# PinataFarms/DAD-3DHeads

Hardware: NVIDIA B200
Metric: heads/sec @256x256 (5023-vert FLAME) (higher is better)
Workload: dtype fp32 operands as fp16 hi/lo split (22-bit), 3 tensor-core products, fp32 accumulate (1e-4 contract met; strict 24-bit mode timed under strict_fp32_operands)

## Files before the change

dad_3dheads_b200/csrc/encoder.cu:

```cuda
#include <algorithm>
#include <cmath>
#include <cstdlib>
#include <cstring>
#include <map>
#include <memory>
#include <string>
#include <vector>

#include "../../include/dad3d.h"
#include "common.h"
#include "encoder_kernels.cuh"
#include "tmap.h"

using namespace dad3d;

namespace {

constexpr int kImg = 256;
constexpr int kStageUnits[4] = {3, 4, 6, 3};
constexpr int kNumFilters = 256;
constexpr int kHeat = 68;
constexpr int kHeatCat = 128;
constexpr int kMlpOut = 549;
constexpr float kLimitValue = 3.0f;
// ... 17 lines not shown
  if (cout <= 80) return 80;
  return 96;
}

inline uint16_t host_bf16(float x) {
  uint32_t u;
  std::memcpy(&u, &x, 4);
  if ((u & 0x7f800000u) == 0x7f800000u) return static_cast<uint16_t>(u >> 16);
  u += 0x7fffu + ((u >> 16) & 1u);
  return static_cast<uint16_t>(u >> 16);
}
inline uint16_t host_f16(float x) { return __half_as_ushort(__float2half_rn(x)); }
inline float host_f16_to_f32(uint16_t b) { return __half2float(__ushort_as_half(b)); }
inline float host_bf16_to_f32(uint16_t b) {
  uint32_t u = static_cast<uint32_t>(b) << 16;
  float f;
  std::memcpy(&f, &u, 4);
  return f;
}

struct TensorInfo {
  int N = 0, H = 0, W = 0, C = 0;
  bool f32 = false;
  int planes = 1;
  size_t bytes = 0;
  int first = 1 << 30, last = -1;
  size_t off = 0;
  uint8_t* ptr = nullptr;
  std::string name;
  long long plane_elems() const { return static_cast<long long>(N) * H * W * C; }
};

enum StepKind { kStemConv, kStemS2d, kStemPool, kConv, kFuse, kConcat, kGap, kFinalize, kHeatExport };

struct Step {
  StepKind kind;
  int in = -1, out = -1, res = -1, out_f32 = -1, in2 = -1, in3 = -1;
  const ConvW* w = nullptr;
  int stride = 1, pad = 0, relu = 0, res_mode = 0, res_stride = 1;
  int up2 = 0;
  int parity = 0;
  int variant = 0;
  int sparse_rows = 0;
  int stem = 0;
  GemmMaps maps;
  GemmGeom geom;
  EpiConv::Params epi;
  float fw[3] = {0, 0, 0};
  int nsrc = 0;
};

struct Plan {
  int B = 0;
  void* ws = nullptr;
  size_t ws_bytes = 0;
  std::vector<TensorInfo> tensors;
  std::vector<Step> steps;
  int t_mlp_out = -1, t_heat = -1, t_c4 = -1;
};

}

struct dad3d_encoder {
  int device = 0;
  int num_sms = 0;
  int P = 3;
  int fp16 = 0;
  int n_mma = 6;
  int n_acc = 2;
  int mma_a[kMaxMma], mma_b[kMaxMma], mma_acc[kMaxMma];
  std::map<std::string, ConvW> convs;
  float* d_stem_w = nullptr;
  float* d_stem_b = nullptr;
  float bifpn_w[2][20];
  std::unique_ptr<Plan> plan;
  size_t ws_cache_B = 0, ws_cache_bytes = 0;
  bool stem_simt = false;
  bool use_halo = true;
  int halo_cluster = 1;
  bool kernels_configured = false, stem_configured = false;
  bool td_parity = false;
  bool heat_sparse = true;
  bool use_pair = false;
  bool use_pdl = false;
  bool debug_keep_all = false;
  bool profile = false;
  std::vector<std::pair<cudaEvent_t, cudaEvent_t>> prof_events;
  size_t prof_used = 0;
  std::vector<const void*> prof_steps;
  double prof_flops = 0.0;
  double prof_bytes = 0.0;
};

namespace {

struct Builder {
  dad3d_encoder* enc;
  Plan* plan;
  int B;

  int tensor(int N, int H, int W, int C, bool f32 = false) {
    TensorInfo t;
    t.N = N; t.H = H; t.W = W; t.C = C; t.f32 = f32;
    t.planes = f32 ? 1 : enc->P;
    t.bytes = align_up(static_cast<size_t>(t.plane_elems()) * (f32 ? 4 : 2) * t.planes, 1024);
    plan->tensors.push_back(t);
    return static_cast<int>(plan->tensors.size()) - 1;
  }
  void touch(int t, int step) {
    if (t < 0) return;
    TensorInfo& ti = plan->tensors[t];
    ti.first = std::min(ti.first, step);
    ti.last = std::max(ti.last, step);
  }
  int push(Step s) {
    const int idx = static_cast<int>(plan->steps.size());
    for (int t : {s.in, s.out, s.res, s.out_f32, s.in2, s.in3}) touch(t, idx);
    plan->steps.push_back(s);
    return idx;
  }
  const ConvW* W(const std::string& name) {
    auto it = enc->convs.find(name);
    return it == enc->convs.end() ? nullptr : &it->second;
  }
  int conv(const std::string& name, int in, int stride, int pad, bool relu, int res = -1, int res_mode = 0,
           bool f32_out = false, bool pieces_out = true, int* f32_id = nullptr, int res_stride = 1, bool up2 = false,
           int variant = 0, int reuse_f32 = -1, bool sparse_rows = false) {
    const ConvW* w = W(name);
    const TensorInfo ti = plan->tensors[in];
    const int Ho = (ti.H + 2 * pad - w->R) / stride + 1;
    const int Wo = (ti.W + 2 * pad - w->S) / stride + 1;
    Step s;
    std::memset(&s.maps, 0, sizeof(s.maps));
    s.kind = kConv;
    s.in = in;
    s.w = w;
    s.stride = stride;
    s.pad = pad;
    s.relu = relu ? 1 : 0;
    s.res = res;
    s.res_mode = res_mode;
    s.res_stride = res_stride;
    s.up2 = up2 ? 1 : 0;
    s.out = pieces_out ? tensor(ti.N, up2 ? 2 * Ho : Ho, up2 ? 2 * Wo : Wo, w->cout_pad) : -1;
    s.out_f32 = f32_out ? (reuse_f32 >= 0 ? reuse_f32 : tensor(ti.N, Ho, Wo, w->cout_pad, true)) : -1;
    s.variant = variant;
    s.sparse_rows = sparse_rows ? 1 : 0;
    if (s.out >= 0) plan->tensors[s.out].name = name;
    if (s.out_f32 >= 0) plan->tensors[s.out_f32].name = name + (pieces_out ? ".f32" : "");
    if (f32_id) *f32_id = s.out_f32;
    push(s);
    return s.out;
  }
};

void pick_tile(int Wo, int Ho, int* tw, int* th, int* tn) {
  int w = 1;
  while (w < Wo && w < kBlockM) w <<= 1;
  *tw = w;
  int h = 1;
  while (h < Ho && w * h < kBlockM) h <<= 1;
  *th = h;
  *tn = kBlockM / (w * h);
}

int build_graph(Builder& b) {
  const int B = b.B;
// ... 202 lines not shown
    const TensorInfo& t = plan->tensors[id];
    v.base = reinterpret_cast<const uint16_t*>(t.ptr);
    v.plane = t.plane_elems();
    v.planes = t.planes;
    v.C = t.C;
    return v;
  };
  for (Step& s : plan->steps) {
    if (s.kind != kConv) continue;
    const TensorInfo& ti = plan->tensors[s.in];
    const ConvW* w = s.w;
    const bool src2 = s.res >= 0 && s.res_mode == 4;
    const int cin2 = src2 ? plan->tensors[s.res].C : 0;
    if (!s.stem && ti.C + cin2 != w->cin_pad) {
      set_error("layer " + w->name + ": input has " + std::to_string(ti.C) + "+" + std::to_string(cin2) +
                " channels, weights expect " + std::to_string(w->cin_pad));
      return DAD3D_ERR_INVALID;
    }
    const int Ho = s.stem ? ti.H : s.parity ? ti.H / 2 : (ti.H + 2 * s.pad - w->R) / s.stride + 1;
    const int Wo = s.stem ? ti.W - kS2dPadW : s.parity ? ti.W / 2 : (ti.W + 2 * s.pad - w->S) / s.stride + 1;
    GemmGeom& g = s.geom;
    std::memset(&g, 0, sizeof(g));
    pick_tile(Wo, Ho, &g.tw, &g.th, &g.tn);
    bool halo = enc->use_halo && !s.stem && w->R == 3 && w->S == 3 && s.stride == 1 && s.pad == 1 && Wo >= kHaloTW &&
                Ho >= kHaloTH;
    if (halo) {
      GemmGeom probe;
      std::memset(&probe, 0, sizeof(probe));
      probe.nA = enc->P; probe.nB = enc->P; probe.block_n = w->block_n;
      halo = gemm_halo_b_stages(probe) >= 2;
    }
    if (s.sparse_rows) halo = false;
    if (halo) { g.tw = kHaloTW; g.th = kHaloTH; g.tn = 1; }
    g.tiles_w = ceil_div(Wo, g.tw);
    g.tiles_h = ceil_div(Ho, g.th);
    if (s.sparse_rows) {
      g.tw = Wo; g.th = 2; g.tn = 1;
      if (g.tw * g.th != kBlockM) { set_error("sparse heat rows need a 64-pixel-wide map"); return DAD3D_ERR_INVALID; }
      g.tiles_w = 1;
      const int Hd = plan->tensors[plan->t_c4].H;
      g.rowmap_n = 0;
      for (int i = 0; i < Hd && g.rowmap_n < 32; ++i) {
        const float fy = (Hd > 1) ? i * (static_cast<float>(Ho - 1) / static_cast<float>(Hd - 1)) : 0.f;
        const int y0 = static_cast<int>(fy);
        if (g.rowmap_n == 0 || g.rowmap[g.rowmap_n - 1] != y0) g.rowmap[g.rowmap_n++] = static_cast<unsigned char>(y0);
      }
      g.tiles_h = g.rowmap_n;
    }
    g.tiles_n = ceil_div(ti.N, g.tn);
    g.Wo = Wo; g.Ho = Ho; g.Nimg = ti.N;
    g.stride = s.stride;
    g.R = w->R; g.S = w->S; g.pad_h = s.pad; g.pad_w = s.pad;
    g.cin_blocks = ti.C / kBlockK;
    if (s.stem) { g.cin_blocks = 1; g.pad_h = 2; g.pad_w = 0; }
    if (s.parity) { g.pad_h = -((s.parity - 1) >> 1); g.pad_w = -((s.parity - 1) & 1); }
    g.cl_m = 1; g.cl_n = 1;
    const bool res_in_k = s.res >= 0 && s.res_mode == 1 && w->has_identity;
    const int m_tiles = g.tiles_w * g.tiles_h * g.tiles_n;
    const bool narrow = w->has_b64 && m_tiles * (w->cout_pad / w->block_n) * 2 <= enc->num_sms;
    const int block_n = narrow ? 64 : w->block_n;
    g.block_n = block_n;
    g.n_tiles = w->cout_pad / block_n;
    g.nA = enc->P; g.nB = enc->P;
    g.n_mma = enc->n_mma;
    g.n_acc = enc->n_acc;
    for (int i = 0; i < enc->n_mma; ++i) { g.mma_a[i] = enc->mma_a[i]; g.mma_b[i] = enc->mma_b[i]; g.mma_acc[i] = enc->mma_acc[i]; }
    g.fmt16 = enc->fp16 ? 0u : 1u;
    if (res_in_k) {
      g.res_kb = block_n / kBlockK;
      g.n_mma_res = enc->P;
      for (int i = 0; i < enc->P; ++i) {
        g.mma_res_a[i] = enc->P - 1 - i;
        g.mma_res_acc[i] = (enc->n_acc == 2 && g.mma_res_a[i] != 0) ? 1 : 0;
      }
    }
    if (src2) {
      g.res_kb = cin2 / kBlockK;
      g.res_kind = 1;
      g.res_stride = s.res_stride;
    }
    const bool pair = enc->use_pair && block_n == 128 && w->has_b64 &&
                      ((m_tiles + 1) / 2) * g.n_tiles >= enc->num_sms / 2;
    g.pair = (pair && !halo) ? 1 : 0;
    g.stages = gemm_max_stages(g);
    if (halo) {
      g.halo = 1;
      if (enc->halo_cluster == 2 && block_n == 128 && w->has_b64 && m_tiles >= 2 * enc->num_sms) {
        g.cl_m = 2;
        g.sched = 1;
      }
      g.stages = 2;
      g.stages_b = gemm_halo_b_stages(g);
      if (g.stages_b < 2) { set_error("layer " + w->name + ": halo pipeline does not fit shared memory"); return DAD3D_ERR_INVALID; }
    }
    if (g.stages < 2) { set_error("layer " + w->name + ": pipeline does not fit shared memory"); return DAD3D_ERR_INVALID; }
    for (int p = 0; p < enc->P; ++p) {
      const uint64_t dims[4] = {static_cast<uint64_t>(s.stem ? kBlockK : ti.C), static_cast<uint64_t>(s.stem ? Wo : ti.W),
                                static_cast<uint64_t>(ti.H), static_cast<uint64_t>(ti.N)};
      const uint64_t strides[3] = {static_cast<uint64_t>(ti.C) * 2, static_cast<uint64_t>(ti.W) * ti.C * 2,
                                   static_cast<uint64_t>(ti.H) * ti.W * ti.C * 2};
      const uint32_t box[4] = {kBlockK, static_cast<uint32_t>(halo ? kHaloPW : g.tw * s.stride),
                               static_cast<uint32_t>(halo ? kHaloPH : g.th * s.stride), static_cast<uint32_t>(g.tn)};
      const uint32_t es[4] = {1, static_cast<uint32_t>(s.stride), static_cast<uint32_t>(s.stride), 1};
      const uint16_t* basep = reinterpret_cast<const uint16_t*>(ti.ptr) + static_cast<size_t>(p) * ti.plane_elems();
      if (!make_tmap_16bit(&s.maps.a[p], basep, 4, dims, strides, box, es)) return DAD3D_ERR_CUDA;
      s.maps.b[p] = (narrow || g.pair || g.cl_m == 2) ? w->map_b64[p] : w->map_b[p];
    }
    if (res_in_k || src2) {
      const TensorInfo& tr = plan->tensors[s.res];
      const int rs = src2 ? s.res_stride : 1;
      for (int p = 0; p < enc->P; ++p) {
        const uint64_t dims[4] = {static_cast<uint64_t>(tr.C), static_cast<uint64_t>(tr.W), static_cast<uint64_t>(tr.H),
                                  static_cast<uint64_t>(tr.N)};
        const uint64_t strides[3] = {static_cast<uint64_t>(tr.C) * 2, static_cast<uint64_t>(tr.W) * tr.C * 2,
                                     static_cast<uint64_t>(tr.H) * tr.W * tr.C * 2};
        const uint32_t box[4] = {kBlockK, static_cast<uint32_t>(g.tw * rs), static_cast<uint32_t>(g.th * rs),
                                 static_cast<uint32_t>(g.tn)};
        const uint32_t es[4] = {1, static_cast<uint32_t>(rs), static_cast<uint32_t>(rs), 1};
        const uint16_t* basep = reinterpret_cast<const uint16_t*>(tr.ptr) + static_cast<size_t>(p) * tr.plane_elems();
        if (!make_tmap_16bit(&s.maps.r[p], basep, 4, dims, strides, box, es)) return DAD3D_ERR_CUDA;
      }
    }
    EpiConv::Params& ep = s.epi;
    std::memset(&ep, 0, sizeof(ep));
    ep.bias = w->d_bias;
    ep.scale = w->d_scale;
    ep.relu = s.relu;
    ep.res_mode = (res_in_k || src2) ? 0 : s.res_mode;
    ep.res = view(s.res);
    ep.up2 = s.up2;
    ep.parity = s.parity;
    if (s.res >= 0 && !src2 && plan->tensors[s.res].C != w->cout_pad) {
      set_error("layer " + w->name + ": residual channel mismatch");
      return DAD3D_ERR_INVALID;
    }
    if (s.out >= 0) {
      const TensorInfo& to = plan->tensors[s.out];
      ep.out = reinterpret_cast<uint16_t*>(to.ptr);
      ep.out_plane = to.plane_elems();
      ep.out_planes = to.planes;
      ep.ld_out = to.C;
      if (block_n != 64 && block_n != 128) {
        set_error("layer " + w->name + ": piece outputs need block_n 64 or 128");
        return DAD3D_ERR_INVALID;
      }
      const int nc = 32;
      const int bw = std::min(g.tw, 32);
      const int bh = std::min(g.th, 32 / bw);
      const int bn = 32 / (bw * bh);
      for (int p = 0; p < to.planes; ++p) {
        uint16_t* basep = reinterpret_cast<uint16_t*>(to.ptr) + static_cast<size_t>(p) * to.plane_elems();
        if (s.up2 || s.parity) {
          const uint64_t C2 = static_cast<uint64_t>(to.C) * 2;
          const uint64_t dims[5] = {static_cast<uint64_t>(to.C), 2, static_cast<uint64_t>(Wo), 2,
                                    static_cast<uint64_t>(to.N) * Ho};
          const uint64_t strides[4] = {C2, 2 * C2, static_cast<uint64_t>(to.W) * C2, 2 * static_cast<uint64_t>(to.W) * C2};
          const uint32_t box[5] = {static_cast<uint32_t>(nc), 1, static_cast<uint32_t>(bw), 1, static_cast<uint32_t>(bh * bn)};
          if (!make_tmap_16bit(&s.maps.c[p], basep, 5, dims, strides, box, nullptr, nc * 2)) return DAD3D_ERR_CUDA;
          continue;
        }
        const uint64_t dims[4] = {static_cast<uint64_t>(to.C), static_cast<uint64_t>(to.W), static_cast<uint64_t>(to.H),
                                  static_cast<uint64_t>(to.N)};
        const uint64_t strides[3] = {static_cast<uint64_t>(to.C) * 2, static_cast<uint64_t>(to.W) * to.C * 2,
                                     static_cast<uint64_t>(to.H) * to.W * to.C * 2};
        const uint32_t box[4] = {static_cast<uint32_t>(nc), static_cast<uint32_t>(bw), static_cast<uint32_t>(bh),
                                 static_cast<uint32_t>(bn)};
// ... 46 lines not shown
      cudaEvent_t a, b;
      DAD3D_CUDA_OK(cudaEventCreate(&a));
      DAD3D_CUDA_OK(cudaEventCreate(&b));
      enc->prof_events.emplace_back(a, b);
    }
    if (enc->prof_steps.size() <= enc->prof_used) enc->prof_steps.resize(enc->prof_used + 1);
    enc->prof_steps[enc->prof_used] = &s;
    ev = &enc->prof_events[enc->prof_used++];
    enc->prof_flops += conv_useful_flops(s);
    DAD3D_CUDA_OK(cudaEventRecord(ev->first, stream));
  }
  {
    cudaLaunchConfig_t cfg{};
    cfg.gridDim = dim3(grid);
    cfg.blockDim = dim3(kGemmThreads);
    cfg.dynamicSmemBytes = gemm_smem_bytes(g);
    cfg.stream = stream;
    cudaLaunchAttribute attr[2];
    int na = 0;
    if (enc->use_pdl) {
      attr[na].id = cudaLaunchAttributeProgrammaticStreamSerialization;
      attr[na].val.programmaticStreamSerializationAllowed = 1;
      ++na;
    }
    if (csz > 1) {
      attr[na].id = cudaLaunchAttributeClusterDimension;
      attr[na].val.clusterDim.x = static_cast<unsigned>(csz);
      attr[na].val.clusterDim.y = 1;
      attr[na].val.clusterDim.z = 1;
      ++na;
    }
    cfg.attrs = attr;
    cfg.numAttrs = na;
    if (g.pair) {
      if (enc->fp16) DAD3D_CUDA_OK(cudaLaunchKernelEx(&cfg, tile_gemm_kernel<EpiConvH, true>, s.maps, g, s.epi));
      else DAD3D_CUDA_OK(cudaLaunchKernelEx(&cfg, tile_gemm_kernel<EpiConv, true>, s.maps, g, s.epi));
    } else {
      if (enc->fp16) DAD3D_CUDA_OK(cudaLaunchKernelEx(&cfg, tile_gemm_kernel<EpiConvH>, s.maps, g, s.epi));
      else DAD3D_CUDA_OK(cudaLaunchKernelEx(&cfg, tile_gemm_kernel<EpiConv>, s.maps, g, s.epi));
    }
  }
  count_launch();
  if (ev) DAD3D_CUDA_OK(cudaEventRecord(ev->second, stream));
  DAD3D_CUDA_OK(cudaGetLastError());
  return DAD3D_OK;
}

}

extern "C" {

int dad3d_encoder_create(dad3d_encoder** out, const dad3d_conv_weights* layers, int32_t n_layers,
                         const float* bifpn_fusion_w_h, int32_t pieces, int32_t operand_format, int32_t device) {
  DAD3D_REQUIRE(out && layers && bifpn_fusion_w_h, "null pointer");
  DAD3D_REQUIRE(pieces >= 1 && pieces <= 3, "pieces must be 1 (one product), 2 (hi/lo, 3 products) or 3 (bf16x3, 6 products)");
  DAD3D_REQUIRE(operand_format == DAD3D_OPERAND_BF16 || (operand_format == DAD3D_OPERAND_FP16 && pieces <= 2),
                "operand_format must be DAD3D_OPERAND_BF16, or DAD3D_OPERAND_FP16 with 1 or 2 pieces");
  DAD3D_CUDA_OK(cudaSetDevice(device));
  cudaDeviceProp prop;
  DAD3D_CUDA_OK(cudaGetDeviceProperties(&prop, device));
  if (prop.major != 10) {
    set_error("libdad3d requires an sm_100 (Blackwell) device");
    return DAD3D_ERR_UNSUPPORTED;
  }
  std::unique_ptr<dad3d_encoder> enc(new dad3d_encoder());
  enc->device = device;
  enc->num_sms = prop.multiProcessorCount;
  enc->P = pieces;
  enc->fp16 = operand_format == DAD3D_OPERAND_FP16 ? 1 : 0;
  if (pieces == 1) {
    enc->n_mma = 1; enc->n_acc = 1; enc->mma_a[0] = 0; enc->mma_b[0] = 0; enc->mma_acc[0] = 0;
  } else if (pieces == 2) {
    const int pa[3] = {1, 0, 0}, pb[3] = {0, 1, 0}, pc[3] = {1, 1, 0};
    enc->n_mma = 3; enc->n_acc = 2;
    for (int i = 0; i < 3; ++i) { enc->mma_a[i] = pa[i]; enc->mma_b[i] = pb[i]; enc->mma_acc[i] = pc[i]; }
  } else {
    const int pa[6] = {2, 0, 1, 1, 0, 0}, pb[6] = {0, 2, 1, 0, 1, 0}, pc[6] = {1, 1, 1, 1, 1, 0};
    enc->n_mma = 6; enc->n_acc = 2;
    for (int i = 0; i < 6; ++i) { enc->mma_a[i] = pa[i]; enc->mma_b[i] = pb[i]; enc->mma_acc[i] = pc[i]; }
  }
  std::memcpy(enc->bifpn_w, bifpn_fusion_w_h, sizeof(enc->bifpn_w));
  {
    const char* e = std::getenv("DAD3D_PDL");
    enc->use_pdl = (e && e[0] == '1');
    const char* e4 = std::getenv("DAD3D_HALO");
    enc->use_halo = !(e4 && e4[0] == '0');
    const char* e5 = std::getenv("DAD3D_HALO_CLUSTER");
    enc->halo_cluster = (e5 && e5[0] == '2') ? 2 : 1;
    const char* e6 = std::getenv("DAD3D_TD_PARITY");
    enc->td_parity = (e6 && e6[0] == '1');
    const char* e9 = std::getenv("DAD3D_HEAT_SPARSE");
    enc->heat_sparse = !(e9 && std::atoi(e9) == 0);
    const char* e3 = std::getenv("DAD3D_PAIR");
    enc->use_pair = (e3 && e3[0] == '1');
    const char* e2 = std::getenv("DAD3D_STEM_SIMT");
    enc->stem_simt = (e2 && e2[0] == '1');
  }

  auto fail = [&](int code) { dad3d_encoder_destroy(enc.release()); return code; };
  std::vector<float> stem_w4;
  for (int li = 0; li < n_layers; ++li) {
    dad3d_conv_weights L = layers[li];
    if (!L.name || !L.weight_h || !L.bias_h || L.cout <= 0 || L.cin <= 0 || L.R <= 0 || L.S <= 0) {
      set_error("invalid layer record " + std::to_string(li));
      return fail(DAD3D_ERR_INVALID);
    }
    const std::string name(L.name);
    if (name == "stem") {
      if (L.cout != 64 || L.cin != 3 || L.R != 7 || L.S != 7) { set_error("stem must be 7x7 3->64"); return fail(DAD3D_ERR_INVALID); }
      std::vector<float> w(147 * 64);
      for (int o = 0; o < 64; ++o)
        for (int r = 0; r < 7; ++r)
          for (int s = 0; s < 7; ++s)
            for (int c = 0; c < 3; ++c)
              w[((c * 7 + r) * 7 + s) * 64 + o] = L.weight_h[((static_cast<size_t>(o) * 7 + r) * 7 + s) * 3 + c];
      if (cudaMalloc(&enc->d_stem_w, w.size() * 4) != cudaSuccess || cudaMalloc(&enc->d_stem_b, 64 * 4) != cudaSuccess ||
          cudaMemcpy(enc->d_stem_w, w.data(), w.size() * 4, cudaMemcpyHostToDevice) != cudaSuccess ||
          cudaMemcpy(enc->d_stem_b, L.bias_h, 64 * 4, cudaMemcpyHostToDevice) != cudaSuccess) {
        set_error("stem upload failed");
        return fail(DAD3D_ERR_CUDA);
      }
      stem_w4.assign(static_cast<size_t>(64) * 4 * 64, 0.f);
      for (int o = 0; o < 64; ++o)
        for (int r = 0; r < 4; ++r)
          for (int dx = 0; dx < 4; ++dx)
            for (int py = 0; py < 2; ++py)
              for (int px = 0; px < 2; ++px) {
                const int ky = 2 * r + py - 1, kx = 2 * dx + px - 1;
                if (ky < 0 || ky > 6 || kx < 0 || kx > 6) continue;
                for (int c = 0; c < 3; ++c)
                  stem_w4[(static_cast<size_t>(o) * 4 + r) * 64 + dx * 16 + (py * 2 + px) * 3 + c] =
                      L.weight_h[((static_cast<size_t>(o) * 7 + ky) * 7 + kx) * 3 + c];
              }
      L.weight_h = stem_w4.data();
      L.cin = 64; L.R = 4; L.S = 1;
    }
    ConvW cw;
    cw.name = name;
    cw.cout = L.cout; cw.cin = L.cin; cw.R = L.R; cw.S = L.S;
    cw.block_n = pick_block_n(L.cout);
    cw.cout_pad = ceil_div(L.cout, cw.block_n) * cw.block_n;
    cw.cin_pad = ceil_div(L.cin, kBlockK) * kBlockK;
    cw.has_identity = name.size() > 4 && L.R == 1 && L.S == 1 &&
                      ((name.compare(name.size() - 2, 2, "c3") == 0 && name.compare(name.size() - 4, 4, "u1c3") != 0) ||
                       name.compare(name.size() - 2, 2, "td") == 0);
    const size_t ktot_main = static_cast<size_t>(L.R) * L.S * cw.cin_pad;
    const size_t ktot = ktot_main + (cw.has_identity ? cw.cout_pad : 0);
    const size_t plane = static_cast<size_t>(cw.cout_pad) * ktot;
    std::vector<uint16_t> packed(plane * pieces, 0);
    std::vector<float> scale(cw.cout_pad, 1.f), up(cw.cout_pad, 1.f);
    if (enc->fp16)
      for (int o = 0; o < L.cout; ++o) {
        float amax = 0.f;
        const float* row = L.weight_h + static_cast<size_t>(o) * L.R * L.S * L.cin;
        for (size_t i = 0; i < static_cast<size_t>(L.R) * L.S * L.cin; ++i) amax = std::max(amax, std::fabs(row[i]));
        int e = 0;
        if (amax > 0.f && std::isfinite(amax)) {
          std::frexp(amax, &e);
          e = std::min(15, 15 - e);
          e = std::max(e, -100);
        }
        up[o] = std::ldexp(1.f, e);
        scale[o] = std::ldexp(1.f, -e);
      }
    if (cw.has_identity)
      for (int o = 0; o < cw.cout_pad; ++o)
        packed[static_cast<size_t>(o) * ktot + ktot_main + o] = enc->fp16 ? host_f16(up[o]) : static_cast<uint16_t>(0x3F80);
    for (int o = 0; o < L.cout; ++o)
      for (int t = 0; t < L.R * L.S; ++t)
        for (int c = 0; c < L.cin; ++c) {
          float r = L.weight_h[(static_cast<size_t>(o) * L.R * L.S + t) * L.cin + c] * up[o];
          const size_t idx = static_cast<size_t>(o) * ktot + static_cast<size_t>(t) * cw.cin_pad + c;
          for (int p = 0; p < pieces; ++p) {
            const uint16_t h = enc->fp16 ? host_f16(r) : host_bf16(r);
            packed[p * plane + idx] = h;
            r -= enc->fp16 ? host_f16_to_f32(h) : host_bf16_to_f32(h);
          }
// ... 288 lines not shown
```

dad_3dheads_b200/csrc/tile_gemm.cuh:

```cuda
#pragma once
#include "ptx.cuh"

namespace dad3d {

constexpr int kBlockM = 128;
constexpr int kBlockK = 64;
constexpr int kTileABytes = kBlockM * kBlockK * 2;
constexpr int kMaxPieces = 3;
constexpr int kMaxMma = 6;
constexpr int kEpiWarps = 8;
constexpr int kFirstEpiWarp = 2;
constexpr int kGemmThreads = (kFirstEpiWarp + kEpiWarps) * 32;
constexpr int kTmemCols = 512;
constexpr int kStageOutBytes = 4096;
constexpr int kGemmSmemLimit = 227 * 1024;
constexpr int kHaloTW = 8, kHaloTH = 16, kHaloPW = kHaloTW + 2, kHaloPH = kHaloTH + 2;
constexpr int kHaloBytes = kHaloPW * kHaloPH * kBlockK * 2;
constexpr int kHaloPieceBytes = 23 * 1024;

struct GemmGeom {
  int tw, th, tn;
  int tiles_w, tiles_h, tiles_n;
  int Wo, Ho, Nimg;
  int stride;
  int R, S, pad_h, pad_w;
  int cin_blocks;
  int n_tiles;
  int block_n;
  int nA, nB;
  int n_mma;
  int mma_a[kMaxMma], mma_b[kMaxMma];
  int n_acc;
  int mma_acc[kMaxMma];
  int res_kb;
  int res_kind;
  int res_stride;
  int n_mma_res;
  int mma_res_a[kMaxPieces], mma_res_acc[kMaxPieces];
  int stages;
  unsigned fmt16;
  int cl_m, cl_n;
  int halo;
  int stages_b;
  int pair;
  int rowmap_n;
  unsigned char rowmap[32];
  int sched;
};

struct GemmMaps {
  CUtensorMap a[kMaxPieces];
  CUtensorMap b[kMaxPieces];
  CUtensorMap c[kMaxPieces];
  CUtensorMap r[kMaxPieces];
};

__host__ __device__ inline int gemm_stage_bytes(const GemmGeom& g) {
  return g.nA * kTileABytes + g.nB * (g.block_n >> g.pair) * kBlockK * 2;
}
__host__ __device__ inline int gemm_halo_a_stage_bytes(const GemmGeom& g) { return g.nA * kHaloPieceBytes; }
__host__ __device__ inline int gemm_b_stage_bytes(const GemmGeom& g) { return g.nB * g.block_n * kBlockK * 2; }
__host__ inline int gemm_fixed_smem_bytes(int extra = 0) {
  return kEpiWarps * kStageOutBytes + extra + 1024  + 512 ;
}
__host__ inline int gemm_max_stages(const GemmGeom& g, int extra = 0) {
  int s = (kGemmSmemLimit - gemm_fixed_smem_bytes(extra)) / gemm_stage_bytes(g);
  return s > 8 ? 8 : s;
}
__host__ inline int gemm_halo_b_stages(const GemmGeom& g, int a_stages = 2) {
  int s = (kGemmSmemLimit - gemm_fixed_smem_bytes(0) - a_stages * gemm_halo_a_stage_bytes(g)) / gemm_b_stage_bytes(g);
  return s > 8 ? 8 : s;
}
__host__ inline int gemm_smem_bytes(const GemmGeom& g, int extra = 0) {
  if (g.halo) return g.stages * gemm_halo_a_stage_bytes(g) + g.stages_b * gemm_b_stage_bytes(g) + gemm_fixed_smem_bytes(extra);
  return g.stages * gemm_stage_bytes(g) + gemm_fixed_smem_bytes(extra);
}

struct TileCoord {
  int m_tile, n_tile;
  int n0, h0, w0;
};

__device__ __forceinline__ TileCoord decode_tile(const GemmGeom& g, int m_tile, int n_tile) {
  TileCoord c;
  c.n_tile = n_tile;
  c.m_tile = m_tile;
  int iw = c.m_tile % g.tiles_w;
  int ih = (c.m_tile / g.tiles_w) % g.tiles_h;
  int in = c.m_tile / (g.tiles_w * g.tiles_h);
  c.n0 = in * g.tn;
  c.h0 = g.rowmap_n > 0 ? static_cast<int>(g.rowmap[ih]) : ih * g.th;
  c.w0 = iw * g.tw;
  return c;
}

__device__ __forceinline__ bool tile_at(const GemmGeom& g, int i, TileCoord* tc) {
  const int m_tiles = g.tiles_w * g.tiles_h * g.tiles_n;
  int m, n;
  if (g.pair) {
    const int t = static_cast<int>(blockIdx.x >> 1) + i * static_cast<int>(gridDim.x >> 1);
    if (t >= ((m_tiles + 1) >> 1) * g.n_tiles) return false;
    n = t % g.n_tiles;
    m = (t / g.n_tiles) * 2 + static_cast<int>(ptx::cluster_ctarank());
  } else if (g.sched == 0) {
    const int t = static_cast<int>(blockIdx.x) + i * static_cast<int>(gridDim.x);
    if (t >= m_tiles * g.n_tiles) return false;
    n = t % g.n_tiles;
    m = t / g.n_tiles;
  } else if (g.cl_m * g.cl_n == 1) {
    m = static_cast<int>(blockIdx.x) + (i / g.n_tiles) * static_cast<int>(gridDim.x);
    if (m >= m_tiles) return false;
    n = i % g.n_tiles;
  } else {
    const int csize = g.cl_m * g.cl_n;
    const int rank = static_cast<int>(ptx::cluster_ctarank());
    const int n_super = (g.n_tiles + g.cl_n - 1) / g.cl_n;
    const int m_super = (m_tiles + g.cl_m - 1) / g.cl_m;
    const int ms = static_cast<int>(blockIdx.x) / csize + (i / n_super) * (static_cast<int>(gridDim.x) / csize);
    if (ms >= m_super) return false;
    m = ms * g.cl_m + rank / g.cl_n;
    n = (i % n_super) * g.cl_n + rank % g.cl_n;
  }
  *tc = decode_tile(g, m, n);
  return true;
}

struct EpiCtx {
  const GemmGeom* g;
  const GemmMaps* maps;
  TileCoord tc;
  int wq;
  int grp;
  int lane;
  uint32_t t_acc;
  uint8_t* stage;
  uint8_t* extra;
  int prev_m_tile;
  mutable int store_seq;
  uint64_t* tempty;
  uint32_t tempty_cluster;
  int n, h, w;
  bool valid;
  long long pix;
  int col0;
  int bw0, bh0, bn0;
};

template <int OFF, int N>
__device__ __forceinline__ void epi_load32(const EpiCtx& c, int c0, float (&x)[N]) {
  static_assert(OFF + 32 <= N, "slice out of range");
  float v[32];
  ptx::tmem_ld_32x32b_x32_f(c.t_acc + static_cast<uint32_t>(c0), v);
  if (c.g->n_acc == 2) {
    float v2[32];
    ptx::tmem_ld_32x32b_x32_f(c.t_acc + static_cast<uint32_t>(c.g->block_n + c0), v2);
    ptx::tmem_ld_wait();
#pragma unroll
    for (int j = 0; j < 32; ++j) x[OFF + j] = v[j] + v2[j];
  } else {
    ptx::tmem_ld_wait();
#pragma unroll
    for (int j = 0; j < 32; ++j) x[OFF + j] = v[j];
  }
}
template <int OFF, int N>
__device__ __forceinline__ void epi_load16(const EpiCtx& c, int c0, float (&x)[N]) {
  static_assert(OFF + 16 <= N, "slice out of range");
  float v[16];
  ptx::tmem_ld_32x32b_x16_f(c.t_acc + static_cast<uint32_t>(c0), v);
  if (c.g->n_acc == 2) {
    float v2[16];
    ptx::tmem_ld_32x32b_x16_f(c.t_acc + static_cast<uint32_t>(c.g->block_n + c0), v2);
    ptx::tmem_ld_wait();
#pragma unroll
    for (int j = 0; j < 16; ++j) x[OFF + j] = v[j] + v2[j];
  } else {
    ptx::tmem_ld_wait();
#pragma unroll
    for (int j = 0; j < 16; ++j) x[OFF + j] = v[j];
  }
}
__device__ __forceinline__ void epi_release_tmem(const EpiCtx& c) {
  ptx::tc_fence_before();
  if (c.tempty_cluster) ptx::mbar_arrive_cluster(c.tempty_cluster);
  else ptx::mbar_arrive(c.tempty);
}
__device__ __forceinline__ void epi_chunk_range(const GemmGeom& g, int grp, int* cb, int* ce) {
  const int nch = (g.block_n + 31) / 32;
  const int per = (nch + 1) / 2;
  *cb = grp * per;
  *ce = min(nch, *cb + per);
}

template <class Epi, bool kPair = false>
__global__ void __launch_bounds__(kGemmThreads, 1)
tile_gemm_kernel(const __grid_constant__ GemmMaps maps, const GemmGeom g, const typename Epi::Params ep) {
  extern __shared__ uint8_t smem_raw[];
  uint8_t* smem = smem_raw + ((1024u - (ptx::smem_u32(smem_raw) & 1023u)) & 1023u);
  const int stage_bytes = g.halo ? gemm_halo_a_stage_bytes(g) : gemm_stage_bytes(g);
  const int b_stage_bytes = gemm_b_stage_bytes(g);
  uint8_t* smem_b = smem + g.stages * stage_bytes;
  uint8_t* out_stage = smem_b + (g.halo ? g.stages_b * b_stage_bytes : 0);
  uint8_t* extra_smem = out_stage + kEpiWarps * kStageOutBytes;
  uint64_t* bars = reinterpret_cast<uint64_t*>(extra_smem + Epi::kExtraSmemBytes);
  uint64_t* full_bar = bars;
  uint64_t* empty_bar = bars + g.stages;
  uint64_t* tfull_bar = bars + 2 * g.stages;
  uint64_t* tempty_bar = tfull_bar + 2;
  uint32_t* tmem_slot = reinterpret_cast<uint32_t*>(tempty_bar + 2);
  uint64_t* bfull_bar = tempty_bar + 3;
  uint64_t* bempty_bar = bfull_bar + 8;

  const int warp = __shfl_sync(0xffffffffu, static_cast<int>(threadIdx.x >> 5), 0);
  const int lane = threadIdx.x & 31;
  const int num_kb = g.R * g.S * g.cin_blocks;

  if (warp == 0 && lane == 0) {
    for (int i = 0; i < g.nA; ++i) ptx::prefetch_tmap(&maps.a[i]);
    for (int i = 0; i < g.nB; ++i) ptx::prefetch_tmap(&maps.b[i]);
  }
  if (warp == 1 && lane == 0) {
    const int n_peers = g.cl_m + g.cl_n - 1;
    for (int s = 0; s < g.stages; ++s) {
      ptx::mbar_init(&full_bar[s], 1);
      ptx::mbar_init(&empty_bar[s], (kPair || g.halo) ? 1 : n_peers);
    }
    if (g.halo)
      for (int s = 0; s < g.stages_b; ++s) {
        ptx::mbar_init(&bfull_bar[s], 1);
        ptx::mbar_init(&bempty_bar[s], g.cl_m);
      }
    for (int b = 0; b < 2; ++b) {
      ptx::mbar_init(&tfull_bar[b], 1);
      ptx::mbar_init(&tempty_bar[b], (kPair ? 2 : 1) * kEpiWarps * 32);
    }
    ptx::fence_mbar_init();
  }
  if (warp == 0) {
    if constexpr (kPair) {
      ptx::tmem_alloc_2sm(tmem_slot, kTmemCols);
      ptx::tmem_relinquish_2sm();
    } else {
      ptx::tmem_alloc(tmem_slot, kTmemCols);
      ptx::tmem_relinquish();
    }
  }
  ptx::tc_fence_before();
  __syncthreads();
  ptx::tc_fence_after();
  const uint32_t tmem_base = *tmem_slot;
  const int csize = kPair ? 2 : g.cl_m * g.cl_n;
  const int crank = csize > 1 ? static_cast<int>(ptx::cluster_ctarank()) : 0;
  const int ci = crank / g.cl_n, cj = crank % g.cl_n;
  uint16_t mask_a = 0, mask_b = 0;
  for (int j = 0; j < g.cl_n; ++j) mask_a |= static_cast<uint16_t>(1u << (ci * g.cl_n + j));
  for (int i = 0; i < g.cl_m; ++i) mask_b |= static_cast<uint16_t>(1u << (i * g.cl_n + cj));
  const uint16_t mask_peers = mask_a | mask_b;
  if (csize > 1) ptx::cluster_sync_all();
  ptx::grid_dep_launch();
  ptx::grid_dep_wait();

  if (warp == 0) {
    if (g.halo) {
      int sa = 0, sbi = 0;
      uint32_t pha = 0, phb = 0;
      auto issue_a = [&](const TileCoord& t, int cb) {
        ptx::mbar_wait(&empty_bar[sa], pha ^ 1u);
        if (ptx::elect_one_sync()) {
          ptx::mbar_expect_tx(&full_bar[sa], static_cast<uint32_t>(g.nA * kHaloBytes));
          for (int i = 0; i < g.nA; ++i)
            ptx::tma_load_4d(smem + sa * stage_bytes + i * kHaloPieceBytes, &maps.a[i], &full_bar[sa], cb * kBlockK, t.w0 - 1,
                             t.h0 - 1, t.n0);
        }
        __syncwarp();
// ... 49 lines not shown
              uint8_t* sb2 = st + g.nA * kTileABytes;
              if (g.res_kind == 0) {
                if (crank == 0)
                  ptx::mbar_expect_tx(&full_bar[stage], static_cast<uint32_t>(2 * (g.nA * kTileABytes + b_half)));
                const int rc = tc.n_tile * g.block_n + r * kBlockK;
                for (int i = 0; i < g.nA; ++i)
                  ptx::tma_load_4d_2sm(st + i * kTileABytes, &maps.r[i], lead_full, rc, tc.w0, tc.h0, tc.n0);
                ptx::tma_load_2d_2sm(sb2, &maps.b[0], lead_full, num_kb * kBlockK + rc, b_row);
              } else {
                if (crank == 0) ptx::mbar_expect_tx(&full_bar[stage], 2 * tx_bytes);
                for (int i = 0; i < g.nA; ++i)
                  ptx::tma_load_4d_2sm(st + i * kTileABytes, &maps.r[i], lead_full, r * kBlockK, tc.w0 * g.res_stride,
                                       tc.h0 * g.res_stride, tc.n0);
                for (int i = 0; i < g.nB; ++i)
                  ptx::tma_load_2d_2sm(sb2 + i * b_half, &maps.b[i], lead_full, (num_kb + r) * kBlockK, b_row);
              }
            } else if (g.res_kind == 0) {
              ptx::mbar_expect_tx(&full_bar[stage], static_cast<uint32_t>(g.nA * kTileABytes + g.block_n * kBlockK * 2));
              const int rc = tc.n_tile * g.block_n + r * kBlockK;
              for (int i = 0; i < g.nA; ++i)
                ptx::tma_load_4d(st + i * kTileABytes, &maps.r[i], &full_bar[stage], rc, tc.w0, tc.h0, tc.n0);
              ptx::tma_load_2d(st + g.nA * kTileABytes, &maps.b[0], &full_bar[stage], num_kb * kBlockK + rc,
                               tc.n_tile * g.block_n);
            } else {
              ptx::mbar_expect_tx(&full_bar[stage], tx_bytes);
              for (int i = 0; i < g.nA; ++i)
                ptx::tma_load_4d(st + i * kTileABytes, &maps.r[i], &full_bar[stage], r * kBlockK, tc.w0 * g.res_stride,
                                 tc.h0 * g.res_stride, tc.n0);
              uint8_t* sb2 = st + g.nA * kTileABytes;
              for (int i = 0; i < g.nB; ++i)
                ptx::tma_load_2d(sb2 + i * g.block_n * kBlockK * 2, &maps.b[i], &full_bar[stage], (num_kb + r) * kBlockK,
                                 tc.n_tile * g.block_n);
            }
            }
            __syncwarp();
            if (++stage == g.stages) { stage = 0; phase ^= 1u; }
            continue;
          }
          const int tap = kb / g.cin_blocks;
          const int cb = kb - tap * g.cin_blocks;
          const int r = tap / g.S;
          const int s = tap - r * g.S;
          ptx::mbar_wait(&empty_bar[stage], phase ^ 1u);
          uint8_t* st = smem + stage * stage_bytes;
          const int cw = tc.w0 * g.stride + s - g.pad_w;
          const int ch = tc.h0 * g.stride + r - g.pad_h;
          uint8_t* sb = st + g.nA * kTileABytes;
          const int kcol = kb * kBlockK;
          if (ptx::elect_one_sync()) {
          if (!kPair) ptx::mbar_expect_tx(&full_bar[stage], tx_bytes);
          else if (crank == 0) ptx::mbar_expect_tx(&full_bar[stage], 2 * tx_bytes);
          if constexpr (kPair) {
            const uint32_t lead_full = ptx::mapa_u32(&full_bar[stage], 0);
            const int b_half = (g.block_n >> 1) * kBlockK * 2;
            for (int i = 0; i < g.nA; ++i)
              ptx::tma_load_4d_2sm(st + i * kTileABytes, &maps.a[i], lead_full, cb * kBlockK, cw, ch, tc.n0);
            for (int i = 0; i < g.nB; ++i)
              ptx::tma_load_2d_2sm(sb + i * b_half, &maps.b[i], lead_full, kcol,
                                   tc.n_tile * g.block_n + crank * (g.block_n >> 1));
          } else if (csize == 1) {
            for (int i = 0; i < g.nA; ++i)
              ptx::tma_load_4d(st + i * kTileABytes, &maps.a[i], &full_bar[stage], cb * kBlockK, cw, ch, tc.n0);
            for (int i = 0; i < g.nB; ++i)
              ptx::tma_load_2d(sb + i * g.block_n * kBlockK * 2, &maps.b[i], &full_bar[stage], kcol,
                               tc.n_tile * g.block_n);
          } else {
            const int a_rows = kBlockM / g.cl_n, b_rows = g.block_n / g.cl_m;
            for (int i = 0; i < g.nA; ++i)
              ptx::tma_load_4d_mc(st + i * kTileABytes + cj * a_rows * kBlockK * 2, &maps.a[i], &full_bar[stage],
                                  cb * kBlockK, cw + cj * a_rows, ch, tc.n0, mask_a);
            for (int i = 0; i < g.nB; ++i)
              ptx::tma_load_2d_mc(sb + i * g.block_n * kBlockK * 2 + ci * b_rows * kBlockK * 2, &maps.b[i],
                                  &full_bar[stage], kcol, tc.n_tile * g.block_n + ci * b_rows, mask_b);
          }
          }
          __syncwarp();
          if (++stage == g.stages) { stage = 0; phase ^= 1u; }
        }
      }
    }
  } else if (warp == 1) {
    if (!kPair || crank == 0) {
      const uint32_t idesc = ptx::make_idesc_f16(g.fmt16, kPair ? 2 * kBlockM : kBlockM, static_cast<uint32_t>(g.block_n));
      const int b_piece_bytes = (g.block_n >> (kPair ? 1 : 0)) * kBlockK * 2;
      int stage = 0;
      uint32_t phase = 0;
      int acc = 0;
      uint32_t acc_phase = 0;
      TileCoord tc_unused;
      int sbi = 0;
      uint32_t phb = 0;
      for (int ti = 0; g.halo && tile_at(g, ti, &tc_unused); ++ti) {
        ptx::mbar_wait(&tempty_bar[acc], acc_phase ^ 1u);
        ptx::tc_fence_after();
        const uint32_t d_tmem = tmem_base + static_cast<uint32_t>(acc * g.n_acc * g.block_n);
        uint32_t started = 0;
        for (int cb = 0; cb < g.cin_blocks; ++cb) {
          ptx::mbar_wait(&full_bar[stage], phase);
          const uint32_t sa = ptx::smem_u32(smem + stage * stage_bytes);
          for (int tap = 0; tap < 9; ++tap) {
            ptx::mbar_wait(&bfull_bar[sbi], phb);
            ptx::tc_fence_after();
            const uint32_t sb = ptx::smem_u32(smem_b + sbi * b_stage_bytes);
            const uint32_t a_off = static_cast<uint32_t>(((tap / 3) * kHaloPW + (tap % 3)) * kBlockK * 2);
            for (int i = 0; i < g.n_mma; ++i) {
              const uint64_t adesc = ptx::make_kmajor_sw128_desc_sbo(sa + g.mma_a[i] * kHaloPieceBytes + a_off,
                                                                     kHaloPW * kBlockK * 2);
              const uint64_t bdesc = ptx::make_kmajor_sw128_desc(sb + g.mma_b[i] * g.block_n * kBlockK * 2);
              const uint32_t a_id = static_cast<uint32_t>(g.mma_acc[i]);
              const uint32_t d_acc = d_tmem + a_id * static_cast<uint32_t>(g.block_n);
              const uint32_t first = (started >> a_id) & 1u;
              started |= 1u << a_id;
              if (ptx::elect_one_sync()) {
#pragma unroll
                for (int k = 0; k < kBlockK / 16; ++k)
                  ptx::umma_f16(d_acc, adesc + 2u * k, bdesc + 2u * k, idesc, k > 0 ? 1u : first);
              }
              __syncwarp();
            }
            if (ptx::elect_one_sync()) {
              if (csize == 1) ptx::umma_commit(&bempty_bar[sbi]);
              else ptx::umma_commit_mc(&bempty_bar[sbi], mask_b);
              if (tap == 8) ptx::umma_commit(&empty_bar[stage]);
              if (tap == 8 && cb == g.cin_blocks - 1) ptx::umma_commit(&tfull_bar[acc]);
            }
            __syncwarp();
            if (++sbi == g.stages_b) { sbi = 0; phb ^= 1u; }
          }
          if (++stage == g.stages) { stage = 0; phase ^= 1u; }
        }
        acc ^= 1;
        if (acc == 0) acc_phase ^= 1u;
      }
      for (int ti = 0; !g.halo && tile_at(g, ti, &tc_unused); ++ti) {
        ptx::mbar_wait(&tempty_bar[acc], acc_phase ^ 1u);
        ptx::tc_fence_after();
        const uint32_t d_tmem = tmem_base + static_cast<uint32_t>(acc * g.n_acc * g.block_n);
        uint32_t started = 0;
        for (int kb = 0; kb < num_kb + g.res_kb; ++kb) {
          ptx::mbar_wait(&full_bar[stage], phase);
          ptx::tc_fence_after();
          const uint32_t sa = ptx::smem_u32(smem + stage * stage_bytes);
          const uint32_t sb = sa + g.nA * kTileABytes;
          const bool res_block = kb >= num_kb && g.res_kind == 0;
          const int n_prod = res_block ? g.n_mma_res : g.n_mma;
          for (int i = 0; i < n_prod; ++i) {
            const int pa = res_block ? g.mma_res_a[i] : g.mma_a[i];
            const int pb = res_block ? 0 : g.mma_b[i];
            const uint64_t adesc = ptx::make_kmajor_sw128_desc(sa + pa * kTileABytes);
            const uint64_t bdesc = ptx::make_kmajor_sw128_desc(sb + pb * b_piece_bytes);
            const uint32_t a_id = static_cast<uint32_t>(res_block ? g.mma_res_acc[i] : g.mma_acc[i]);
            const uint32_t d_acc = d_tmem + a_id * static_cast<uint32_t>(g.block_n);
            const uint32_t first = (started >> a_id) & 1u;
            started |= 1u << a_id;
            if (ptx::elect_one_sync()) {
#pragma unroll
              for (int k = 0; k < kBlockK / 16; ++k) {
                if constexpr (kPair) ptx::umma_f16_2sm(d_acc, adesc + 2u * k, bdesc + 2u * k, idesc, k > 0 ? 1u : first);
                else ptx::umma_f16(d_acc, adesc + 2u * k, bdesc + 2u * k, idesc, k > 0 ? 1u : first);
              }
            }
            __syncwarp();
          }
          const bool last_kb = kb == num_kb + g.res_kb - 1;
          if (ptx::elect_one_sync()) {
            if constexpr (kPair) ptx::umma_commit_2sm_mc(&empty_bar[stage], 3);
            else if (csize == 1) ptx::umma_commit(&empty_bar[stage]);
            else ptx::umma_commit_mc(&empty_bar[stage], mask_peers);
            if (last_kb) {
              if constexpr (kPair) ptx::umma_commit_2sm_mc(&tfull_bar[acc], 3);
              else ptx::umma_commit(&tfull_bar[acc]);
            }
          }
          __syncwarp();
          if (++stage == g.stages) { stage = 0; phase ^= 1u; }
        }
        acc ^= 1;
        if (acc == 0) acc_phase ^= 1u;
      }
    }
  } else if (warp >= kFirstEpiWarp) {
    typename Epi::State user_state;
    EpiCtx c;
    c.g = &g;
    c.maps = &maps;
    c.wq = warp & 3;
    c.grp = (warp - kFirstEpiWarp) >> 2;
    c.lane = lane;
    c.stage = out_stage + (warp - kFirstEpiWarp) * kStageOutBytes;
    c.extra = extra_smem;
    c.prev_m_tile = -1;
    c.store_seq = 0;
    const int row = c.wq * 32 + lane;
    const int iw = row % g.tw;
    const int ih = (row / g.tw) % g.th;
    const int in = row / (g.tw * g.th);
    const int row0 = c.wq * 32;
    const int biw = row0 % g.tw, bih = (row0 / g.tw) % g.th, bin = row0 / (g.tw * g.th);
    int acc = 0;
    uint32_t acc_phase = 0;
    for (int ti = 0; tile_at(g, ti, &c.tc); ++ti) {
      c.n = c.tc.n0 + in;
      c.h = c.tc.h0 + ih;
      c.w = c.tc.w0 + iw;
      c.valid = (c.n < g.Nimg) && (c.h < g.Ho) && (c.w < g.Wo);
      c.pix = (static_cast<long long>(c.n) * g.Ho + c.h) * g.Wo + c.w;
      c.col0 = c.tc.n_tile * g.block_n;
      c.bw0 = c.tc.w0 + biw;
      c.bh0 = c.tc.h0 + bih;
      c.bn0 = c.tc.n0 + bin;
      c.tempty = &tempty_bar[acc];
      c.tempty_cluster = kPair ? ptx::mapa_u32(&tempty_bar[acc], 0) : 0u;
      c.t_acc = tmem_base + (static_cast<uint32_t>(c.wq * 32) << 16) + static_cast<uint32_t>(acc * g.n_acc * g.block_n);
      Epi::prefetch(ep, c, user_state);
      ptx::mbar_wait(&tfull_bar[acc], acc_phase);
      ptx::tc_fence_after();
      Epi::run(ep, c, user_state);
      c.prev_m_tile = c.tc.m_tile;
      acc ^= 1;
      if (acc == 0) acc_phase ^= 1u;
    }
    if (lane == 0) ptx::bulk_wait_read0();
  }

  ptx::tc_fence_before();
  __syncthreads();
  if (csize > 1) ptx::cluster_sync_all();
  if (warp == 0) {
    ptx::tc_fence_after();
    if constexpr (kPair) ptx::tmem_dealloc_2sm(tmem_base, kTmemCols);
    else ptx::tmem_dealloc(tmem_base, kTmemCols);
  }
}

}
```

Before: 14440.

## Merge the last two split-precision UMMAs into one wide-N MMA and enable PDL

When the last two tensor-core products share the same A piece and write to adjacent B pieces and accumulators, they are now issued as a single MMA with twice the N width. Only the first k-slice is kept as two separate MMAs, because its accumulate flags can differ. This cuts the number of issued UMMA instructions and makes better use of the wide-N shape. Programmatic dependent launch is also switched on by default, to overlap kernel launch prologues. The merge depends on B pieces and TMEM accumulators being contiguous, and enabling PDL by default may expose ordering hazards.

```diff
diff --git a/dad_3dheads_b200/csrc/encoder.cu b/dad_3dheads_b200/csrc/encoder.cu
--- a/dad_3dheads_b200/csrc/encoder.cu
+++ b/dad_3dheads_b200/csrc/encoder.cu
@@ -123,7 +123,8 @@
   bool td_parity = false;
   bool heat_sparse = true;
   bool use_pair = false;
-  bool use_pdl = false;
+  bool merge_mma = true;
+  bool use_pdl = true;
   bool debug_keep_all = false;
   bool profile = false;
   std::vector<std::pair<cudaEvent_t, cudaEvent_t>> prof_events;
@@ -492,6 +493,11 @@
     const bool pair = enc->use_pair && block_n == 128 && w->has_b64 &&
                       ((m_tiles + 1) / 2) * g.n_tiles >= enc->num_sms / 2;
     g.pair = (pair && !halo) ? 1 : 0;
+    const int l = g.n_mma - 2;
+    g.merge_last2 = (enc->merge_mma && !s.stem && g.n_acc == 2 && l >= 0 && g.mma_a[l] == g.mma_a[l + 1] &&
+                     g.mma_b[l] == 1 && g.mma_acc[l] == 1 && g.mma_b[l + 1] == 0 && g.mma_acc[l + 1] == 0 &&
+                     2 * block_n <= 256 && !g.pair)
+                        ? 1 : 0;
     g.stages = gemm_max_stages(g);
     if (halo) {
       g.halo = 1;
@@ -704,7 +710,7 @@
   std::memcpy(enc->bifpn_w, bifpn_fusion_w_h, sizeof(enc->bifpn_w));
   {
     const char* e = std::getenv("DAD3D_PDL");
-    enc->use_pdl = (e && e[0] == '1');
+    enc->use_pdl = !(e && e[0] == '0');
     const char* e4 = std::getenv("DAD3D_HALO");
     enc->use_halo = !(e4 && e4[0] == '0');
     const char* e5 = std::getenv("DAD3D_HALO_CLUSTER");
@@ -715,6 +721,8 @@
     enc->heat_sparse = !(e9 && std::atoi(e9) == 0);
     const char* e3 = std::getenv("DAD3D_PAIR");
     enc->use_pair = (e3 && e3[0] == '1');
+    const char* e7 = std::getenv("DAD3D_MERGE_MMA");
+    enc->merge_mma = !(e7 && e7[0] == '0');
     const char* e2 = std::getenv("DAD3D_STEM_SIMT");
     enc->stem_simt = (e2 && e2[0] == '1');
   }
diff --git a/dad_3dheads_b200/csrc/tile_gemm.cuh b/dad_3dheads_b200/csrc/tile_gemm.cuh
--- a/dad_3dheads_b200/csrc/tile_gemm.cuh
+++ b/dad_3dheads_b200/csrc/tile_gemm.cuh
@@ -32,6 +32,7 @@
   int mma_a[kMaxMma], mma_b[kMaxMma];
   int n_acc;
   int mma_acc[kMaxMma];
+  int merge_last2;
   int res_kb;
   int res_kind;
   int res_stride;
@@ -190,6 +191,20 @@
   const int per = (nch + 1) / 2;
   *cb = grp * per;
   *ce = min(nch, *cb + per);
+}
+
+__device__ __forceinline__ void umma_merged_pair(uint32_t d_tmem, uint32_t block_n, uint64_t adesc, uint64_t bdesc0,
+                                                 uint64_t bdesc1, uint32_t idesc, uint32_t idesc2, uint32_t accum0,
+                                                 uint32_t accum1) {
+#pragma unroll
+  for (int k = 0; k < kBlockK / 16; ++k) {
+    if (k == 0 && accum0 != accum1) {
+      ptx::umma_f16(d_tmem + block_n, adesc, bdesc1, idesc, accum1);
+      ptx::umma_f16(d_tmem, adesc, bdesc0, idesc, accum0);
+    } else {
+      ptx::umma_f16(d_tmem, adesc + 2u * k, bdesc0 + 2u * k, idesc2, k > 0 ? 1u : accum0);
+    }
+  }
 }
 
 template <class Epi, bool kPair = false>
@@ -405,6 +420,8 @@
   } else if (warp == 1) {
     if (!kPair || crank == 0) {
       const uint32_t idesc = ptx::make_idesc_f16(g.fmt16, kPair ? 2 * kBlockM : kBlockM, static_cast<uint32_t>(g.block_n));
+      const uint32_t idesc2 = ptx::make_idesc_f16(g.fmt16, kBlockM, 2u * static_cast<uint32_t>(g.block_n));
+      const bool merge = !kPair && g.merge_last2;
       const int b_piece_bytes = (g.block_n >> (kPair ? 1 : 0)) * kBlockK * 2;
       int stage = 0;
       uint32_t phase = 0;
@@ -434,6 +451,17 @@
               const uint32_t d_acc = d_tmem + a_id * static_cast<uint32_t>(g.block_n);
               const uint32_t first = (started >> a_id) & 1u;
               started |= 1u << a_id;
+              if constexpr (!kPair) {
+                if (merge && i == g.n_mma - 2) {
+                  const uint32_t first0 = started & 1u;
+                  started |= 1u;
+                  if (ptx::elect_one_sync())
+                    umma_merged_pair(d_tmem, static_cast<uint32_t>(g.block_n), adesc, ptx::make_kmajor_sw128_desc(sb), bdesc,
+                                     idesc, idesc2, first0, first);
+                  __syncwarp();
+                  break;
+                }
+              }
               if (ptx::elect_one_sync()) {
 #pragma unroll
                 for (int k = 0; k < kBlockK / 16; ++k)
@@ -476,6 +504,17 @@
             const uint32_t d_acc = d_tmem + a_id * static_cast<uint32_t>(g.block_n);
             const uint32_t first = (started >> a_id) & 1u;
             started |= 1u << a_id;
+            if constexpr (!kPair) {
+              if (merge && !res_block && i == n_prod - 2) {
+                const uint32_t first0 = started & 1u;
+                started |= 1u;
+                if (ptx::elect_one_sync())
+                  umma_merged_pair(d_tmem, static_cast<uint32_t>(g.block_n), adesc, ptx::make_kmajor_sw128_desc(sb), bdesc,
+                                   idesc, idesc2, first0, first);
+                __syncwarp();
+                break;
+              }
+            }
             if (ptx::elect_one_sync()) {
 #pragma unroll
               for (int k = 0; k < kBlockK / 16; ++k) {
```

New measurement: 14890 (median of 6 runs). +3.1%, better.
